# chenghuailin/trajectory_optimization_matrix_lie_groups

Measured on AMD Instinct MI355X. Metric: DDP iterations/sec at batch x horizon = 4096 x 200 (SE3 tracking), higher is better.
Workload: dtype f64

## Files before the change

### trajectory_optimization_matrix_lie_groups_amd/csrc/tolg_backward3.h

```cpp
template <int M>
__host__ __device__ constexpr int urow(int u) { return (u < 3 || M == 6) ? 6 + u : 11; }

#ifndef TOLG_DPP_BUILTIN
#define DF3(acc, p, q, L) "v_fmac_f64_dpp " acc ", " p ", " q " row_newbcast:" L " row_mask:0xf bank_mask:0xf\n\t"
template <int M, int J, int LN>
TOLG_DEV void ldl3_update(double (&a)[M], double w) {
  constexpr int R = M - 1 - J;
  if constexpr (J == 0) {
    if constexpr (M == 6)
      asm volatile("s_nop 1" : "+v"(a[1]), "+v"(a[2]), "+v"(a[3]), "+v"(a[4]), "+v"(a[5]));
    else
      asm volatile("s_nop 1" : "+v"(a[1]), "+v"(a[2]), "+v"(a[3]));
  }
  if constexpr (R == 5)
    asm volatile(DF3("%0", "%0", "%5", "%6") DF3("%1", "%1", "%5", "%6") DF3("%2", "%2", "%5", "%6")
                     DF3("%3", "%3", "%5", "%6") DF3("%4", "%4", "%5", "%6")
                 : "+v"(a[J + 1]), "+v"(a[J + 2]), "+v"(a[J + 3]), "+v"(a[J + 4]), "+v"(a[J + 5]) : "v"(w), "n"(LN));
  if constexpr (R == 4)
    asm volatile(DF3("%0", "%0", "%4", "%5") DF3("%1", "%1", "%4", "%5") DF3("%2", "%2", "%4", "%5")
                     DF3("%3", "%3", "%4", "%5")
                 : "+v"(a[J + 1]), "+v"(a[J + 2]), "+v"(a[J + 3]), "+v"(a[J + 4]) : "v"(w), "n"(LN));
  if constexpr (R == 3)
    asm volatile(DF3("%0", "%0", "%3", "%4") DF3("%1", "%1", "%3", "%4") DF3("%2", "%2", "%3", "%4")
                 : "+v"(a[J + 1]), "+v"(a[J + 2]), "+v"(a[J + 3]) : "v"(w), "n"(LN));
// ... 120 lines not shown
  ldl3_tie_columns<M>(a);
  zn[0] = y[0] * nri[0];
  if constexpr (M > 1) { ldl3_fwd_row<M, 1, LO>(y[1], a[1], zn); zn[1] = y[1] * nri[1]; }
  if constexpr (M > 2) { ldl3_fwd_row<M, 2, LO>(y[2], a[2], zn); zn[2] = y[2] * nri[2]; }
  if constexpr (M > 3) { ldl3_fwd_row<M, 3, LO>(y[3], a[3], zn); zn[3] = y[3] * nri[3]; }
  if constexpr (M > 4) { ldl3_fwd_row<M, 4, LO>(y[4], a[4], zn); zn[4] = y[4] * nri[4]; }
  if constexpr (M > 5) { ldl3_fwd_row<M, 5, LO>(y[5], a[5], zn); zn[5] = y[5] * nri[5]; }
}
template <int M, int LO = 0>
TOLG_DEV void ldl3_backward_nx(const double (&a)[M], const double (&nri)[M], double (&y)[M], const double (&zn)[M], double (&nx)[M]) {
  nx[M - 1] = zn[M - 1];
  if constexpr (M > 1) { ldl3_bwd_row<M, M - 2, urow<M>(M - 2) + LO>(y[M - 2], a, nx); nx[M - 2] = y[M - 2] * nri[M - 2]; }
  if constexpr (M > 2) { ldl3_bwd_row<M, M - 3, urow<M>(M - 3) + LO>(y[M - 3], a, nx); nx[M - 3] = y[M - 3] * nri[M - 3]; }
  if constexpr (M > 3) { ldl3_bwd_row<M, M - 4, urow<M>(M - 4) + LO>(y[M - 4], a, nx); nx[M - 4] = y[M - 4] * nri[M - 4]; }
  if constexpr (M > 4) { ldl3_bwd_row<M, M - 5, urow<M>(M - 5) + LO>(y[M - 5], a, nx); nx[M - 5] = y[M - 5] * nri[M - 5]; }
  if constexpr (M > 5) { ldl3_bwd_row<M, M - 6, urow<M>(M - 6) + LO>(y[M - 6], a, nx); nx[M - 6] = y[M - 6] * nri[M - 6]; }
}

enum { B3_DATA = 5120, B3_ZBYTES = 256,
       B3_ID = B3_DATA + B3_ZBYTES, B3_IDBYTES = 6 * 192, B3_SLOT = B3_ID + B3_IDBYTES,
       B3_TRS = 14, B3_TR = 2 * B3_SLOT, B3_TRBYTES = 4 * 12 * B3_TRS * 8, B3_DUMP = B3_TR + B3_TRBYTES,
       B3_KC = B3_DUMP + 12 * B3_TRS * 8, B3_LDS = B3_KC + 16 * 16 * 8 };

template <int M, bool GRAV, bool AL, bool FAST = false, bool PTW = false>
__global__ __launch_bounds__(64) void k_backward3(Params P, int it, int flags) {
  if ((flags & 4) && !P.k2_redo[blockIdx.x]) return;
  const int ms = flags & 1;
  const bool closed = (flags & 2) != 0;
  const DConsts& C = *(const DConsts*)P.c;
  const int lane = threadIdx.x, g = lane >> 4, j = lane & 15;
  const int b = blockIdx.x * 4 + g;
  const bool act = P.active[b] != 0;
  if constexpr (FAST) {
    const bool back = __any(act && P.mu[b] != 0.0) || P.k2_hint[blockIdx.x] != 0;
    if (lane == 0) P.k2_redo[blockIdx.x] = back ? 1 : 0;
    if (back) return;
  }
  if (!__any(act)) return;
  const int N = P.N;
  __shared__ __attribute__((aligned(16))) char lds[FAST ? (B3_LDS > 34 * 1024 ? B3_LDS : 34 * 1024) : B3_LDS];
  if (lane < B3_ZBYTES / 8) {
    reinterpret_cast<double*>(lds + B3_DATA)[lane] = 0.0;
    reinterpret_cast<double*>(lds + B3_SLOT + B3_DATA)[lane] = 0.0;
  }
  for (int k = lane; k < B3_IDBYTES / 8; k += 64) {
    const int c6 = k / 24, w = k % 24, pr = w / 8, hf = w % 8;
    const double v = (hf < 2 && 2 * pr + hf == c6) ? 1.0 : 0.0;
    reinterpret_cast<double*>(lds + B3_ID)[k] = v;
    reinterpret_cast<double*>(lds + B3_SLOT + B3_ID)[k] = v;
  }
  __builtin_amdgcn_wave_barrier();
  const unsigned lds0 = (unsigned)(uintptr_t)(__attribute__((address_space(3))) char*)lds;

  const double m12 = (j < 12) ? 1.0 : 0.0;
  int mycol = -1;
#pragma unroll
  for (int u = 0; u < M; u++) if (j == urow<M>(u)) mycol = u;
  double bu[M], ibu[M];
#pragma unroll
  for (int u = 0; u < M; u++) { bu[u] = fu_entry<M>(*P.c, urow<M>(u) - 6, u); ibu[u] = 1.0 / bu[u]; }
  double kBW[6], Rt[M], wm[M];
  if constexpr (PTW) {
    const double wd = (j >= 6 && j < 12) ? C.wts[(size_t)(WT_W2 + (j >= 6 && j < 12 ? j - 6 : 0)) * P.Bp + b] : 0.0;
#pragma unroll
    for (int r = 0; r < 6; r++) kBW[r] = (j >= 6 && j < 12) ? 2.0 * (r == j - 6 ? wd : 0.0) : 0.0;
  } else {
#pragma unroll
    for (int r = 0; r < 6; r++) kBW[r] = (j >= 6 && j < 12) ? 2.0 * C.W2[6 * r + (j - 6)] : 0.0;
  }
  {
    double ibc = 0.0;
#pragma unroll
    for (int u = 0; u < M; u++) if (mycol == u) ibc = ibu[u];
    const double rd = (PTW && mycol >= 0) ? C.wts[(size_t)(WT_R + (mycol >= 0 ? mycol : 0)) * P.Bp + b] : 0.0;
#pragma unroll
    for (int u = 0; u < M; u++) {
      Rt[u] = (mycol >= 0) ? 2.0 * (PTW ? (u == mycol ? rd : 0.0) : C.R[u * M + (mycol >= 0 ? mycol : 0)]) * ibu[u] * ibc : 0.0;
      wm[u] = (mycol > u) ? 1.0 : 0.0;
    }
  }
  int fT = REC_D, fM = REC_D + 3;
  bool hT = false, hM = false;
  if (j < 3) { fT = REC_RI + 3 * j; fM = REC_TRI + 3 * j; hT = true; hM = true; }
  else if (j < 6) { fM = REC_RI + 3 * (j - 3); hM = true; }
  else if (j < 9) { fT = REC_JR + 3 * (j - 6); fM = REC_QR + 3 * (j - 6); hT = true; hM = true; }
  else if (j < 12) { fM = REC_JR + 3 * (j - 9); hM = true; }
  else if (j == 12 && !closed) { hT = true; hM = true; }
  const bool vcol = j >= 6 && j < 12;
  const bool hasB = (j == 12 && !closed), isVec = (j == 12 || j == 13);
  const int fB = REC_D + 6;
  const bool hL = (j < 6 || isVec);
  const unsigned lg = (unsigned)g * 16u;
  const unsigned ZP = (unsigned)B3_DATA;
  unsigned oT[3], oM[3], oL[6];
#pragma unroll
  for (int r = 0; r < 3; r++) { oT[r] = hT ? lg + FOFF(fT + r) : ZP; oM[r] = hM ? lg + FOFF(fM + r) : ZP; }
#pragma unroll
  for (int r = 0; r < 6; r++) oL[r] = hL ? lg + FOFF((j < 6) ? REC_LXX + sym6(r, j) : REC_LX + r) : ZP;
  const unsigned oB = hasB ? lg + FOFF(fB) : vcol ? (unsigned)B3_ID + (unsigned)(j - 6) * 192u : ZP;
  unsigned oXA = lg + FOFF(REC_XI), oXB = oXA;
  {
    double aA[2] = {0, 0}, bA[2] = {0, 0}, aB[2] = {0, 0}, bB[2] = {0, 0}, mA[3] = {0, 0, 0}, mB[3] = {0, 0, 0};
    if (vcol) {
      const Consts& G = *P.c;
      const int Cb = (j - 6) / 3, cc = (j - 6) % 3, kA = (cc + 1) % 3, kB = (cc + 2) % 3;
      auto sg = [](int r, int c) { return ((c - r + 3) % 3 == 1) ? -1.0 : 1.0; };
      const double dt = G.dt, ms = G.mass;
      const double iaA = G.Ibinv[4 * kA], iaB = G.Ibinv[4 * kB], icA = G.Jvinv[4 * kA], icB = G.Jvinv[4 * kB];
      const double a_kA = G.Ib[4 * kA], a_kB = G.Ib[4 * kB], a_cc = G.Ib[4 * cc], c_cc = G.Jv[4 * cc];
      const double sA = sg(kA, cc), sB_ = sg(kB, cc);
      if (so3_family(G.kind)) {
        if (Cb == 0) { aA[0] = dt * iaA * sA * (a_kB - a_cc); aB[0] = dt * iaB * sB_ * (a_kA - a_cc); }
      } else if (Cb == 0) {
        aA[0] = dt * iaA * sA * a_kB; bA[0] = -dt * iaA * sA * a_cc;
        aB[0] = dt * iaB * sB_ * a_kA; bB[0] = -dt * iaB * sB_ * a_cc;
        bA[1] = dt * icA * sA * ms; bB[1] = dt * icB * sB_ * ms;
      } else {
        aA[0] = -dt * iaA * sA * c_cc; bA[0] = dt * iaA * sA * ms;
        aB[0] = -dt * iaB * sB_ * c_cc; bB[0] = dt * iaB * sB_ * ms;
        bA[1] = -dt * icA * sA * c_cc; bB[1] = -dt * icB * sB_ * c_cc;
      }
      mA[kA] = 1.0; mB[kB] = 1.0;
      oXA = lg + FOFF(REC_XI + 2 * kA); oXB = lg + FOFF(REC_XI + 2 * kB);
    }
    if (g == 0) {
      double* kc = reinterpret_cast<double*>(lds + B3_KC) + 16 * j;
      kc[0] = aA[0]; kc[1] = bA[0]; kc[2] = aB[0]; kc[3] = bB[0]; kc[4] = bA[1]; kc[5] = bB[1];
#pragma unroll
      for (int r = 0; r < 3; r++) { kc[6 + 2 * r] = mA[r]; kc[7 + 2 * r] = mB[r]; }
    }
  }
  const unsigned oKC = (unsigned)B3_KC + 128u * (unsigned)j;
  const unsigned oV = isVec ? lg + FOFF(REC_LX + 6) : ZP;
  const unsigned oU = isVec ? lg + FOFF(REC_LU) : ZP;
  const unsigned oG = lg + FOFF(REC_LU + M);
  constexpr bool al = AL;
  constexpr unsigned blockBytes = (unsigned)rec_fields(M, GRAV, AL, false) * 32u;
  constexpr int NKB = (int)((blockBytes + 1023u) / 1024u);
  static_assert(NKB == 3 || NKB == 4, "record block of four trajectories: 3 or 4 KB");
  const unsigned oUU = (al && mycol >= 0) ? lg + FOFF(P.fLUU + (mycol >= 0 ? mycol : 0)) : ZP;
  const unsigned wTR = (j < 12) ? (unsigned)B3_TR + ((unsigned)g * 12u * B3_TRS + (unsigned)j) * 8u : (unsigned)B3_DUMP;
  const unsigned rTR = (j < 12) ? (unsigned)B3_TR + ((unsigned)g * 12u * B3_TRS + (unsigned)j * B3_TRS) * 8u : ZP;
  const double hsym = (j < 12) ? 0.5 : 1.0;
  const unsigned sB = (unsigned)P.Bp * 8u;
  const unsigned vr = REC_VR(b);
  const unsigned vG = GK_VG(b, M) + GOFF(0, (j < 13 ? j : 12), M);
  const size_t recStride = (size_t)P.recF * P.Bp, gStride = (size_t)13 * M * P.Bp;
  double Cg[GRAV ? 3 : 1][6];
  if constexpr (GRAV) {
#pragma unroll
    for (int a = 0; a < 3; a++)
#pragma unroll
      for (int r = 0; r < 6; r++) Cg[a][r] = (j < 3) ? C.Llin[a][6 * r + (j < 3 ? j : 0)] : 0.0;
  }
  double mu = P.mu[b], delta = P.delta[b];
  int warned = 0;

  auto dma_from = [&](const char* src, int s) {
    const unsigned dst = (unsigned)__builtin_amdgcn_readfirstlane((int)(lds0 + (unsigned)s * B3_SLOT));
    if constexpr (NKB == 3) rl_dma16x3_rec(uniform_ptr(src), (unsigned)lane * 16u, dst);
    else rl_dma16x4_rec(uniform_ptr(src), (unsigned)lane * 16u, dst);
  };
  auto dma_knot = [&](int i, int s) {
    dma_from(reinterpret_cast<const char*>(P.REC + recStride * i) + (size_t)blockIdx.x * blockBytes, s);
  };
  const char* rec_run = reinterpret_cast<const char*>(P.REC + recStride * (size_t)(N > 2 ? N - 2 : 0)) + (size_t)blockIdx.x * blockBytes;
  const double* gk_run = P.GK + gStride * (size_t)(N + 1);
  const size_t recStrideB = recStride * 8;

  double V[12];
  {
    __amdgpu_buffer_rsrc_t rR = mkbuf(P.REC + recStride * N, (unsigned)P.recF * sB);
    const unsigned OOB = 0x40000000u;
    const double pd = (PTW && j >= 6 && j < 12) ? C.wts[(size_t)(WT_P2 + (j >= 6 && j < 12 ? j - 6 : 0)) * P.Bp + b] : 0.0;
#pragma unroll
    for (int r = 0; r < 6; r++) {
      const int fl = (j < 6) ? REC_LXX + sym6(r, j) : REC_LX + r;
      double t1 = bld(rR, hL ? vr + FOFF(fl) : OOB, 0), t2 = bld(rR, isVec ? vr + FOFF(REC_LX + 6 + r) : OOB, 0);
      V[r] = t1;
      double p2 = (j >= 6 && j < 12) ? 2.0 * (PTW ? (r == j - 6 ? pd : 0.0) : C.P2[6 * r + (j - 6)]) : 0.0;
      V[6 + r] = t2 + p2;
    }
  }
  double gsum = 0;
  double Kst[M];
#pragma unroll
  for (int u = 0; u < M; u++) Kst[u] = 0;
  auto store_gains = [&](const double* gk) {
    if (act && j < 13) {
      __amdgpu_buffer_rsrc_t rGs = mkbuf(gk, 13 * M * sB);
#pragma unroll
      for (int u = 0; u < M; u += 2) bst2_gk(rGs, vG, GOFF(u, 0, M), Kst[u], Kst[u + 1]);
    }
  };
#ifdef TOLG_STAMPS
  unsigned long long st_acc[8] = {0, 0, 0, 0, 0, 0, 0, 0}, st_t = __builtin_amdgcn_s_memtime();
  const unsigned long long st_rt0 = __builtin_amdgcn_s_memrealtime(), st_ct0 = st_t;
#endif

  bool failed = false;
  auto step = [&](int i, auto slot_tag) {
    constexpr int SLOT = decltype(slot_tag)::value;
    const char* sl = lds + SLOT * B3_SLOT;
    auto ld = [&](unsigned off) -> double { return *reinterpret_cast<const double*>(sl + off); };
    auto ld2 = [&](unsigned off, int k, double& x0, double& x1) {
      const f64x2 w = *reinterpret_cast<const f64x2*>(sl + off + k * 64);
      x0 = w.x; x1 = w.y;
    };
    if (i == 0) asm volatile("s_waitcnt vmcnt(0)" ::: "memory");
    else asm volatile("s_waitcnt vmcnt(%0)" :: "n"(M / 2 + NKB) : "memory");
    double A[12], Qh[12], lu[M], luu_i = 0.0;
#pragma unroll
    for (int r = 0; r < 3; r++) { A[r] = ld(oT[r]); A[3 + r] = ld(oM[r]); }
#pragma unroll
    for (int r = 0; r < 6; r += 2) ld2(oB, r / 2, A[6 + r], A[7 + r]);
#pragma unroll
    for (int r = 0; r < 6; r++) Qh[r] = ld(oL[r]);
#pragma unroll
    for (int r = 0; r < 6; r += 2) ld2(oV, r / 2, Qh[6 + r], Qh[7 + r]);
#pragma unroll
    for (int a = 0; a < M; a += 2) ld2(oU, a / 2, lu[a], lu[a + 1]);
    if constexpr (al) luu_i = ld(oUU);
    if constexpr (GRAV) {
      double gv[3];
#pragma unroll
      for (int a = 0; a < 3; a++) gv[a] = *reinterpret_cast<const double*>(sl + oG + (FOFF(REC_LU + M + a) - FOFF(REC_LU + M)));
#pragma unroll
      for (int r = 0; r < 6; r++) A[6 + r] += gv[0] * Cg[0][r] + gv[1] * Cg[1][r] + gv[2] * Cg[2][r];
    }
    const f64x2 xA = *reinterpret_cast<const f64x2*>(sl + oXA), xB = *reinterpret_cast<const f64x2*>(sl + oXB);
    const f64x2* kc = reinterpret_cast<const f64x2*>(lds + oKC);
    const f64x2 c0 = kc[0], c1 = kc[1], c2 = kc[2];
    const f64x2 mk0 = kc[3], mk1 = kc[4], mk2 = kc[5];
    STAMP(0)
    double Z[12];
#pragma unroll
    for (int r = 0; r < 12; r++) Z[r] = (1.0 - m12) * V[r];
    rank1_bk3_0(Z, V, A[0], A[1], A[2]); rank1_bk3_3_nn(Z, V, A[3], A[4], A[5]);
    {
      const double eA0 = fma(c0.x, xB.x, c0.y * xB.y), eB0 = fma(c1.x, xA.x, c1.y * xA.y), eA1 = c2.x * xB.y, eB1 = c2.y * xA.y;
      A[6] = fma(mk0.y, eB0, fma(mk0.x, eA0, A[6])); A[9] = fma(mk0.y, eB1, fma(mk0.x, eA1, A[9]));
      A[7] = fma(mk1.y, eB0, fma(mk1.x, eA0, A[7])); A[10] = fma(mk1.y, eB1, fma(mk1.x, eA1, A[10]));
      A[8] = fma(mk2.y, eB0, fma(mk2.x, eA0, A[8])); A[11] = fma(mk2.y, eB1, fma(mk2.x, eA1, A[11]));
    }
    rank1_bk3_6_nn(Z, V, A[6], A[7], A[8]); rank1_bk3_9_nn(Z, V, A[9], A[10], A[11]);
    STAMP(1)
    __builtin_amdgcn_sched_barrier(0);
    asm volatile("s_waitcnt lgkmcnt(0)" ::: "memory");
#ifdef TOLG_STAMPS2
    STAMP(1)
#endif
    gk_run -= gStride;
    if (i < N - 1) store_gains(gk_run);
#ifdef TOLG_STAMPS2
    STAMP(2)
#endif
    rec_run -= recStrideB;
    if (i >= 2) dma_from(rec_run, SLOT);
    __builtin_amdgcn_sched_barrier(0);
#ifndef TOLG_STAMPS2
    STAMP(2)
#endif
    bool use_lu = false;
    double mu_used = 0.0;
    auto build = [&](double mu_, double (&Gm)[M], double (&Mt)[M]) {
      const double muA = m12 * mu_;
#pragma unroll
      for (int u = 0; u < M; u++) {
        Gm[u] = fma(lu[u], ibu[u], Z[urow<M>(u)]);
        Mt[u] = V[urow<M>(u)] + Rt[u];
      }
      if (__any(mu_ != 0.0)) {
#pragma unroll
        for (int u = 0; u < M; u++) {
          Gm[u] = fma(muA, A[urow<M>(u)], Gm[u]);
          Mt[u] += (mycol == u) ? mu_ : 0.0;
// ... 32 lines not shown
#define TOLG_K3_SYMP 4
#endif
    static_assert(TOLG_K3_SYMP >= 1 && (TOLG_K3_SYMP & (TOLG_K3_SYMP - 1)) == 0, "symmetrisation period: a power of two");
    constexpr int SYMP = FAST ? TOLG_K3_SYMP : 1;
    const bool sym_now = SYMP == 1 || (SLOT == 0 && (SYMP == 2 || (i & (SYMP - 1)) == 0));
    if (sym_now) {
#pragma unroll
      for (int r = 0; r < 12; r++) *reinterpret_cast<double*>(lds + wTR + r * (B3_TRS * 8)) = Qh[r];
    }
    double T[12];
    auto read_T = [&]() {
#pragma unroll
      for (int k = 0; k < 6; k++) {
        const f64x2 t = *reinterpret_cast<const f64x2*>(lds + rTR + 16 * k);
        T[2 * k] = t.x; T[2 * k + 1] = t.y;
      }
    };
    auto symmetrise = [&]() {
      if (!sym_now) return;
      read_T();
#pragma unroll
      for (int r = 0; r < 12; r++) Qh[r] = hsym * (Qh[r] + T[r]);
    };
    auto grad_term = [&](const double (&G)[M]) {
      double s0 = 0, s1 = 0;
#pragma unroll
      for (int u = 0; u < M; u += 2) {
        const double q0 = bu[u] * G[u], q1 = bu[u + 1] * G[u + 1];
        s0 = fma(q0, q0, s0); s1 = fma(q1, q1, s1);
      }
      const double s_ = s0 + s1;
      const double y = __builtin_amdgcn_rsq(s_);
      const double r_ = s_ * y, h_ = 0.5 * y;
      const double rt = fma(h_, fma(-r_, r_, s_), r_);
      gsum += (s_ > 0.0) ? rt : 0.0;
    };
    auto finish = [&](double (&Y)[M], const double (&Uf)[M], double (&nri)[M]) {
      grad_term(Y);
      STAMP(4)
      if (!ms) {
#pragma unroll
        for (int u = 0; u < M; u++) nri[u] = (j == 13) ? 0.0 : nri[u];
      }
      double zn[M], nx[M];
      ldl3_forward<M>(Uf, nri, Y, zn);
      symmetrise();
      STAMP(5)
      if constexpr (M == 6) rank1_bi_x6_nn(Qh, Y, zn);
      else rank1_bi_x4_nn(Qh, Y, zn);
      ldl3_backward_nx<M>(Uf, nri, Y, zn, nx);
#pragma unroll
      for (int u = 0; u < M; u++) Kst[u] = ibu[u] * nx[u];
    };
    bool settled = false;
#ifdef TOLG_K3_NOFAST
    if (false) {
#else
    if (FAST || !__any(act && mu != 0.0)) {
#endif
      double Y[M], Uf[M], nri[M], dv[M];
#pragma unroll
      for (int u = 0; u < M; u++) {
        Y[u] = fma(lu[u], ibu[u], Z[urow<M>(u)]);
        Uf[u] = V[urow<M>(u)] + Rt[u];
        if constexpr (al) Uf[u] += (mycol == u) ? luu_i * ibu[u] * ibu[u] : 0.0;
      }
      ldl3_factor<M>(Uf, nri, dv, wm);
      const bool pd = ldl3_all_positive<M>(dv);
      STAMP(3)
      if (!__any(act && !pd)) {
        if (act) { delta = fmin(1.0, delta) * 0.5; mu = 0.0; }
        finish(Y, Uf, nri);
        settled = true;
      }
    }
    if constexpr (FAST) {
      if (!settled) { failed = true; return; }
    } else if (!settled) {
      double Y2[M], U2[M], nr2[M], d2[M];
      for (;;) {
        if (!done) {
          mu_used = mu;
          build(mu, Y2, U2);
          ldl3_factor<M>(U2, nr2, d2, wm);
          done = schedule(ldl3_all_positive<M>(d2));
        }
        if (__all(done)) break;
      }
      build(mu_used, Y2, U2);
      ldl3_factor<M>(U2, nr2, d2, wm);
      if (!__any(use_lu)) {
        finish(Y2, U2, nr2);
      } else {
        double Gk[M], Mc[M], Ac[M][M], Xl[M], zn[M], nx[M];
        build(mu_used, Gk, Mc);
        grad_term(Gk);
// ... 32 lines not shown
#pragma unroll
        for (int u = 0; u < M; u++) Kst[u] = ibu[u] * (use_lu ? -((j == 13) ? 0.0 : Xl[u]) : nx[u]);
      }
    }
#pragma unroll
    for (int r = 0; r < 12; r++) V[r] = Qh[r];
    STAMP(6)
  };

  dma_knot(N - 1, (N - 1) & 1);
  if (N >= 2) dma_knot(N - 2, (N - 2) & 1);
  asm volatile("s_waitcnt vmcnt(0)" ::: "memory");
  int i = N - 1;
  if (i & 1) { step(i, std::integral_constant<int, 1>()); i--; }
  for (; i >= 1 && !(FAST && failed); i -= 2) {
    step(i, std::integral_constant<int, 0>());
    if (FAST && failed) break;
    step(i - 1, std::integral_constant<int, 1>());
  }
  if (i == 0 && !(FAST && failed)) step(0, std::integral_constant<int, 0>());
  if constexpr (FAST) {
    if (failed) {
      asm volatile("s_waitcnt vmcnt(0)" ::: "memory");
      if (lane == 0) { P.k2_redo[blockIdx.x] = 1; P.k2_hint[blockIdx.x] = 8; }
      return;
    }
  } else {
    const bool anyf = __any(failed);
    if (lane == 0) { const int hn = (it == 0) ? 0 : P.k2_hint[blockIdx.x]; P.k2_hint[blockIdx.x] = anyf ? 8 : (hn > 0 ? hn - 1 : 0); }
  }
  store_gains(P.GK);
#ifdef TOLG_STAMPS
  STAMP(7)
  if (blockIdx.x == 7 && lane == 0 && P.mu_hist) {
    for (int k = 0; k < 8; k++) P.mu_hist[(size_t)28 * P.max_iter + k] = (double)st_acc[k];
    P.mu_hist[(size_t)29 * P.max_iter + 0] = (double)(__builtin_amdgcn_s_memrealtime() - st_rt0);
    P.mu_hist[(size_t)29 * P.max_iter + 1] = (double)(__builtin_amdgcn_s_memtime() - st_ct0);
  }
#endif
  double grad = (ms ? bcast<12>(gsum) : bcast<13>(gsum)) / (double)N;
  if (act && j == 0) {
    P.mu[b] = mu;
    P.delta[b] = delta;
    P.grad[b] = grad;
    if (warned) P.status[b] = TOLG_ST_MAXREG;
    if (it >= 0 && b < P.B) {
      if (P.grad_hist) P.grad_hist[(size_t)b * (P.max_iter + 1) + it] = grad;
      if (P.mu_hist && it < P.max_iter) P.mu_hist[(size_t)b * P.max_iter + it] = mu;
    }
    if (it >= 0) {
      bool conv = ms ? (grad < P.tol_grad && P.dn[b] < P.tol_defect) : (grad < P.tol_grad);
      if (conv) { P.conv[b] = 1; P.active[b] = 0; }
    }
  }
}
```

### trajectory_optimization_matrix_lie_groups_amd/csrc/tolg_kernels.hip

```cpp
#include <hip/hip_runtime.h>
#include <hip/hip_ext.h>
#include <type_traits>
#include <math.h>
#include <stdint.h>
#include <stdio.h>
#include <stdlib.h>
#include <string.h>
#include <new>
#include <vector>

#include "../../include/tolg.h"
#include "tolg_lie.h"

namespace tolg {

struct Consts {
  int kind, m, N, diagJ;
  double dt, mass, grav, pend_k;
  double J[36], Jinv[36], Ib[9];
  double Jv[9], Ibinv[9], Jvinv[9];
  double W1[36], W2[36], P1[36], P2[36];
  double R[36];
  double Bt[9], Bb[9];
  double Llin[3][36];
// ... 3405 lines not shown
  int b = blockIdx.x * blockDim.x + threadIdx.x;
  if (b >= P.B) return;
  if (J) J[b] = P.Jc[b];
  if (dn) dn[b] = P.dn[b];
  if (grad) grad[b] = P.grad[b];
  if (mu_delta) { mu_delta[2 * b] = P.mu[b]; mu_delta[2 * b + 1] = P.delta[b]; }
  if (iters) iters[b] = P.iters[b];
  if (status) status[b] = P.status[b];
  if (conv) conv[b] = P.conv[b];
}

}

using namespace tolg;

typedef void (*SearchKernel)(Params, int, int, int);
typedef void (*SearchRollout)(Params, int, int, int, int);
struct KernelTable {
  void (*init)(Params, const double*, const double*, const double*, int);
  void (*init_warm)(Params, const double*, const double*, const double*, const double*, const double*);
  void (*linearize)(Params, const double*, const double*, double*, double*, int, int, int, int, int);
  void (*init_rollout)(Params);
  void (*sweep[2][2])(Params, int, int);
  void (*rollout_linear)(Params, double, int, int);
  void (*rollout_alpha1)(Params, double, int, int);
  void (*rollout_factor)(Params, double, int, int);
  void (*rollout_lin)(Params, int);
  void (*ec_ring[2])(Params);
  void (*ec_stmt[2])(Params);
  void (*affine_commit)(Params, int, int);
  void (*policy_rollout)(Params, int, int, const double*, const double*, double*, int*, double*, double*, double*);
  void (*mpc_advance)(Params, const double*, double*, double*, double*, double*, double*, double*);
  void (*policy_rollout_plant[2])(Params, int, int, const double*, const double*, double*, int*, double*, double*, double*, PlantArg);
  void (*mpc_advance_plant[2])(Params, const double*, double*, double*, double*, double*, double*, double*, PlantArg);
  struct Search {
    struct { SearchRollout k; int nt; } wave2[2];
    SearchRollout wave1[2];
    SearchKernel eval_t[2];
    SearchKernel eval, eval_affine;
  } ls[2];
};

template <int M, bool MS, int PK, int PT>
static KernelTable::Search search_kernels() {
  KernelTable::Search s;
  s.wave2[1] = {k_rollout_ls2<M, false, 1, PK>, 1};
  if constexpr (MS || PK == 1) s.wave2[0] = {k_rollout_ls2<M, MS, 1, PK>, 1};
  else s.wave2[0] = {k_rollout_ls2<M, false, 3>, 3};
  s.wave1[0] = k_rollout_ls<M, MS, false, PK>;
  s.wave1[1] = k_rollout_ls<M, MS, true, PK>;
  s.eval_t[0] = k_rollout_eval_t<M, MS, false, PT>;
  s.eval_t[1] = k_rollout_eval_t<M, MS, true, PT>;
  s.eval = k_ls_eval<M, MS, PT>;
  s.eval_affine = k_ls_eval_affine<M, MS, PT>;
  return s;
}
template <int M, bool GRAV, bool DENSE, bool PEND, int PT>
static KernelTable kernel_table(int lds_per_block) {
  constexpr int PK = PEND ? 1 : 0;
  constexpr bool PTREF = (PT & PT_REF) != 0, PTW = (PT & PT_W) != 0;
  KernelTable t;
  t.init = k_init<PTREF>;
  t.init_warm = k_init_warm;
  t.linearize = k_linearize<M, PT>;
  t.init_rollout = k_init_rollout<M>;
  if constexpr (!DENSE && !PEND) {
    t.sweep[0][0] = k_backward3<M, GRAV, false, false, PTW>; t.sweep[0][1] = k_backward3<M, GRAV, true, false, PTW>;
    t.sweep[1][0] = k_backward3<M, GRAV, false, true, PTW>;  t.sweep[1][1] = k_backward3<M, GRAV, true, true, PTW>;
  } else {
    t.sweep[0][0] = t.sweep[0][1] = k_backward<M, PEND, GRAV, PEND && !DENSE, false, PTW>;
    t.sweep[1][0] = t.sweep[1][1] = k_backward<M, PEND, GRAV, PEND && !DENSE, true, PTW>;
  }
  t.rollout_linear = k_rollout<M, true, false>;
  t.rollout_alpha1 = k_rollout<M, false, true, PK>;
  t.rollout_factor = k_rollout<M, false, false, PK>;
  t.rollout_lin = nullptr;
  if constexpr (!PEND)
    if (rl_static_lds<M>() + sizeof(double) * RL_NH * 4 * 16 <= (size_t)lds_per_block) t.rollout_lin = k_rollout_lin<M, PT>;
  t.ec_ring[0] = k_expected_change_ring<M, GRAV, false, DENSE || PEND, PEND, PTW>;
  t.ec_ring[1] = k_expected_change_ring<M, GRAV, true, DENSE || PEND, PEND, PTW>;
  t.ec_stmt[0] = k_expected_change<M, PK, false, PTW>;
  t.ec_stmt[1] = k_expected_change<M, PK, true, PTW>;
  t.affine_commit = k_affine_commit<M>;
  t.policy_rollout = k_policy_rollout<M, PK, PT & ~PT_OBS>;
  t.mpc_advance = k_mpc_advance<M, PK, PT & ~PT_OBS>;
  t.policy_rollout_plant[TOLG_PLANT_DIAG] = k_policy_rollout<M, PK, PT & ~PT_OBS, PL_DIAG, PlantArg>;
  t.policy_rollout_plant[TOLG_PLANT_DENSE] = k_policy_rollout<M, PK, PT & ~PT_OBS, PL_DENSE, PlantArg>;
  t.mpc_advance_plant[TOLG_PLANT_DIAG] = k_mpc_advance<M, PK, PT & ~PT_OBS, PL_DIAG, PlantArg>;
  t.mpc_advance_plant[TOLG_PLANT_DENSE] = k_mpc_advance<M, PK, PT & ~PT_OBS, PL_DENSE, PlantArg>;
  t.ls[0] = search_kernels<M, false, PK, PT>();
  t.ls[1] = search_kernels<M, true, PK, PT>();
// ... 60 lines not shown
  Params P;
  Params run;
  tolg_options run_opt;
  LsPlan run_ls;
  int run_it;
  bool running;
  int lds_per_block;
  int rec_closed = 0;
  KernelTable kt;
  KernelTable kt_pt[8];
  const double* ref_shared;
  const double* refs = nullptr;
  int refs_B = 0;
  const double* wts = nullptr;
  int wts_B = 0;
  const double* obs = nullptr;
  int obs_B = 0, obs_K = 0;
  double *obs_lam = nullptr, *obs_imu = nullptr;
  const double* plant = nullptr;
  int plant_B = 0, plant_S = 0, plant_form = 0;
  int pol_B = 0;
  bool pol_traj_fast = false;
  bool k2_full_only, ls_one_wave;
  const double *al_lb, *al_ub, *al_lambda, *al_imu;
  LazyRes cnt;
  LazyRes side;
  bool timing;
  std::vector<hipEvent_t> ev;
  std::vector<int> ev_kind;
  size_t ev_used;
};

static size_t align_up(size_t x, size_t a) { return (x + a - 1) / a * a; }
static int padded_batch(int B) { return (B + 3) / 4 * 4; }
static dim3 traj_grid(const Params& P) { return dim3((P.Bp + 63) / 64); }
static dim3 knot_grid(int knots, int Bp) { return dim3((unsigned)(((size_t)knots * Bp + 255) / 256)); }

static bool batch_fits(const tolg_handle_s* h, int B) {
  return B >= 1 && B <= h->max_batch && !(h->refs && B != h->refs_B) && !(h->wts && B != h->wts_B) && !(h->obs && B != h->obs_B);
}
static void select_kernels(tolg_handle_s* h) {
  h->kt = h->kt_pt[(h->refs ? PT_REF : 0) | (h->wts ? PT_W : 0) | (h->obs ? PT_OBS : 0)];
}

static int host_inv6(const double A[36], double Ai[36]) {
  double Mx[6][12];
// ... 173 lines not shown
        double sacc = 0;
        if (j < 3 && c.grav != 0.0 && prob->kind != TOLG_DYN_PENDULUM3D)
          for (int k = 0; k < 3; k++) sacc += c.Jinv[6 * i + 3 + k] * S[3 * k + j];
        if (j < 3 && i < 3 && prob->kind == TOLG_DYN_PENDULUM3D) {
          const double SS[9] = {c.pend_k * S[3 + 0], c.pend_k * S[3 + 1], c.pend_k * S[3 + 2],
                                -c.pend_k * S[0], -c.pend_k * S[1], -c.pend_k * S[2], 0, 0, 0};
          for (int k = 0; k < 3; k++) sacc += c.Ibinv[3 * i + k] * SS[3 * k + j];
        }
        c.Llin[a][6 * i + j] = sacc * prob->dt;
      }
  }
  h->kt_pt[0] = kernel_table_for<0>(*prob, c, h->lds_per_block);
  h->kt_pt[PT_REF] = kernel_table_for<PT_REF>(*prob, c, h->lds_per_block);
  h->kt_pt[PT_W] = kernel_table_for<PT_W>(*prob, c, h->lds_per_block);
  h->kt_pt[PT_REF | PT_W] = kernel_table_for<PT_REF | PT_W>(*prob, c, h->lds_per_block);
  h->kt_pt[PT_OBS] = kernel_table_for<PT_OBS>(*prob, c, h->lds_per_block);
  h->kt_pt[PT_REF | PT_OBS] = kernel_table_for<PT_REF | PT_OBS>(*prob, c, h->lds_per_block);
  h->kt_pt[PT_W | PT_OBS] = kernel_table_for<PT_W | PT_OBS>(*prob, c, h->lds_per_block);
  h->kt_pt[PT_REF | PT_W | PT_OBS] = kernel_table_for<PT_REF | PT_W | PT_OBS>(*prob, c, h->lds_per_block);
  select_kernels(h);
  {
    const char* e = getenv("TOLG_K2_FULL_ONLY");
    h->k2_full_only = e && e[0] == '1';
    e = getenv("TOLG_LS_ONEWAVE");
    h->ls_one_wave = e && e[0] == '1';
    e = getenv("TOLG_POLICY_TRAJ_FAST");
    h->pol_traj_fast = e && e[0] == '1';
  }
  hipStream_t st = static_cast<hipStream_t>(stream);
  memset(&h->P, 0, sizeof h->P);
  carve_all(prob, h->Bp_max, h->ws, h->P);
  h->P.N = prob->N; h->P.m = prob->m;
  h->ref_shared = h->P.ref;
  Consts* dc = const_cast<Consts*>(h->P.c);
  if (hipMemcpyAsync(dc, &h->hc, sizeof(Consts), hipMemcpyHostToDevice, st) != hipSuccess) { tolg_destroy(h); return TOLG_E_LAUNCH; }
  int N = prob->N;
  hipLaunchKernelGGL(k_pack_ref, dim3((N + 1 + 63) / 64), dim3(64), 0, st, N, d_q_ref, d_xi_ref,
                     const_cast<double*>(h->P.ref));
  LAUNCH_CHECK();
  *out = h;
  return 0;
}

extern "C" void tolg_destroy(tolg_handle_t h) {
  if (!h) return;
  h->cnt.release();
  h->side.release();
  for (auto e : h->ev) (void)hipEventDestroy(e);
  delete h;
}

extern "C" void tolg_enable_timing(tolg_handle_t h, int32_t on) {
  if (!h) return;
  h->timing = on != 0;
  if (h->timing && h->ev.empty()) {
    h->ev.resize(2 * 1024);
    for (auto& e : h->ev) (void)hipEventCreate(&e);
    h->ev_kind.resize(1024);
  }
  h->ev_used = 0;
}

namespace {
struct Timed {
  tolg_handle_s* h; hipStream_t st; int kind; bool on, ext;
  bool count = true;
  Timed(tolg_handle_s* h_, hipStream_t s, int k, bool ext_ = false) : h(h_), st(s), kind(k), ext(ext_) {
    on = h->timing;
// ... 57 lines not shown
  return P;
}

static int run_linearize(tolg_handle_s* h, const Params& P, hipStream_t st, const double* src, const double* src_u,
                         double* dst, double* dst_u, int ms, int i0 = 0, int ni = -1, int ls_list = -1, int ls_nslots = 0,
                         decltype(KernelTable::linearize) kernel = nullptr) {
  if (ni < 0) ni = P.N + 1;
  h->rec_closed = 0;
  Timed t(h, st, 2);
  hipLaunchKernelGGL(kernel ? kernel : h->kt.linearize, knot_grid(ni, P.Bp), dim3(256), 0, st, P, src, src_u, dst, dst_u, ms, i0,
                     ni, ls_list, ls_nslots);
  LAUNCH_CHECK();
  return 0;
}
static int run_backward(tolg_handle_s* h, const Params& P, hipStream_t st, int it, int ms) {
  ms = (ms ? 1 : 0) | (h->rec_closed ? 2 : 0);
  const dim3 grid(P.Bp / 4), blk(64);
  const bool al = P.al_lb != nullptr;
  const bool fast = it > 0 && !h->k2_full_only;
  for (int pass = fast ? 0 : 1; pass < 2; pass++) {
    Timed t(h, st, 0, true);
    t.count = (pass == 0) || !fast;
    const int fl = ms | ((pass == 1 && fast) ? 4 : 0);
    t.launch(h->kt.sweep[pass == 0][al], grid, blk, P, it, fl);
    LAUNCH_CHECK();
  }
  return 0;
}
static int run_rollout_ms(tolg_handle_s* h, const Params& P, hipStream_t st, double alpha, int linear, int ms = 1,
                          int i0 = 0, int i1 = -1) {
  if (i1 < 0) i1 = P.N;
  Timed t(h, st, 1);
  dim3 grid((P.Bp * 4 + 63) / 64), blk(64);
  const KernelTable& T = h->kt;
  hipLaunchKernelGGL(linear ? T.rollout_linear : (alpha == 1.0 || !ms) ? T.rollout_alpha1 : T.rollout_factor, grid, blk, 0,
                     st, P, alpha, i0, i1);
  LAUNCH_CHECK();
  return 0;
}
static void launch_ec_ring(const tolg_handle_s* h, const Params& P, hipStream_t st, bool store) {
  hipLaunchKernelGGL(h->kt.ec_ring[store], dim3(P.Bp / 4), dim3(64), 0, st, P);
}
static void launch_ec_stmt(const tolg_handle_s* h, const Params& P, hipStream_t st, bool redo) {
  hipLaunchKernelGGL(h->kt.ec_stmt[redo], dim3((P.Bp * 4 + 63) / 64), dim3(64), 0, st, P);
}
static int run_affine_dev(tolg_handle_s* h, const Params& P, hipStream_t st, bool merit) {
  Timed t(h, st, 1);
// ... 673 lines not shown
```

Before: 1823.

## Pair fast backward sweep waves with helper waves computing gains via LDS ring

```diff
diff --git a/trajectory_optimization_matrix_lie_groups_amd/csrc/tolg_backward3.h b/trajectory_optimization_matrix_lie_groups_amd/csrc/tolg_backward3.h
--- a/trajectory_optimization_matrix_lie_groups_amd/csrc/tolg_backward3.h
+++ b/trajectory_optimization_matrix_lie_groups_amd/csrc/tolg_backward3.h
@@ -166,35 +166,84 @@
        B3_TRS = 14, B3_TR = 2 * B3_SLOT, B3_TRBYTES = 4 * 12 * B3_TRS * 8, B3_DUMP = B3_TR + B3_TRBYTES,
        B3_KC = B3_DUMP + 12 * B3_TRS * 8, B3_LDS = B3_KC + 16 * 16 * 8 };
 
-template <int M, bool GRAV, bool AL, bool FAST = false, bool PTW = false>
-__global__ __launch_bounds__(64) void k_backward3(Params P, int it, int flags) {
-  if ((flags & 4) && !P.k2_redo[blockIdx.x]) return;
+typedef rl_sync_t b3_sync_t;
+enum { B3_STOP = -1 };
+TOLG_DEV int b3_wait(b3_sync_t p, int v) {
+  int x = *p;
+  for (int n = 0; n < RL_POLLS && x >= 0 && x < v; n++) {
+    __builtin_amdgcn_s_sleep(2);
+    x = *p;
+  }
+  return x;
+}
+template <int M>
+struct B3Ring { enum { ROWS = 3 * M / 2, SLOT = ROWS * 1024, BYTES = 2 * SLOT }; };
+template <int M>
+TOLG_DEV void b3_ring_put_factor(char* rs, const double (&a)[M], const double (&nri)[M], double s_) {
+  f64x2* q = reinterpret_cast<f64x2*>(rs);
+#pragma unroll
+  for (int u = 0; u < M; u += 2) q[(u / 2) * 64] = f64x2{nri[u], nri[u + 1]};
+#pragma unroll
+  for (int u = 1; u < M; u += 2) q[(M / 2 + u / 2) * 64] = f64x2{a[u], u + 1 < M ? a[u + 1 < M ? u + 1 : u] : s_};
+}
+template <int M>
+TOLG_DEV void b3_ring_put_y(char* rs, const double (&Y)[M]) {
+  f64x2* q = reinterpret_cast<f64x2*>(rs);
+#pragma unroll
+  for (int u = 0; u < M; u += 2) q[(M + u / 2) * 64] = f64x2{Y[u], Y[u + 1]};
+}
+TOLG_DEV double b3_grad_root(double s_) {
+  const double y = __builtin_amdgcn_rsq(s_);
+  const double r_ = s_ * y, h_ = 0.5 * y;
+  const double rt = fma(h_, fma(-r_, r_, s_), r_);
+  return (s_ > 0.0) ? rt : 0.0;
+}
+TOLG_DEV void b3_epilogue_grad(const Params& P, int it, int ms, int b, bool act, int j, double gsum) {
+  double grad = (ms ? bcast<12>(gsum) : bcast<13>(gsum)) / (double)P.N;
+  if (act && j == 0) {
+    P.grad[b] = grad;
+    if (it >= 0 && b < P.B && P.grad_hist) P.grad_hist[(size_t)b * (P.max_iter + 1) + it] = grad;
+    if (it >= 0) {
+      bool conv = ms ? (grad < P.tol_grad && P.dn[b] < P.tol_defect) : (grad < P.tol_grad);
+      if (conv) { P.conv[b] = 1; P.active[b] = 0; }
+    }
+  }
+}
+
+struct B3Pair {
+  unsigned ring;
+  b3_sync_t prod, cons;
+};
+template <int M, bool GRAV, bool AL, bool FAST, bool PTW, int ROLE>
+TOLG_DEV void b3_sweep(const Params& P, const int it, const int flags, const int grp, char* const lds, const unsigned wb, const B3Pair pr) {
+  static_assert(ROLE == 0 || FAST, "only the fast sweep has a helper");
+  auto leave = [&]() { if constexpr (ROLE == 1) *pr.prod = B3_STOP; };
+  if ((flags & 4) && !P.k2_redo[grp]) { leave(); return; }
   const int ms = flags & 1;
   const bool closed = (flags & 2) != 0;
   const DConsts& C = *(const DConsts*)P.c;
-  const int lane = threadIdx.x, g = lane >> 4, j = lane & 15;
-  const int b = blockIdx.x * 4 + g;
+  const int lane = threadIdx.x & 63, g = lane >> 4, j = lane & 15;
+  const int b = grp * 4 + g;
   const bool act = P.active[b] != 0;
   if constexpr (FAST) {
-    const bool back = __any(act && P.mu[b] != 0.0) || P.k2_hint[blockIdx.x] != 0;
-    if (lane == 0) P.k2_redo[blockIdx.x] = back ? 1 : 0;
-    if (back) return;
-  }
-  if (!__any(act)) return;
+    const bool back = __any(act && P.mu[b] != 0.0) || P.k2_hint[grp] != 0;
+    if (lane == 0) P.k2_redo[grp] = back ? 1 : 0;
+    if (back) { leave(); return; }
+  }
+  if (!__any(act)) { leave(); return; }
   const int N = P.N;
-  __shared__ __attribute__((aligned(16))) char lds[FAST ? (B3_LDS > 34 * 1024 ? B3_LDS : 34 * 1024) : B3_LDS];
   if (lane < B3_ZBYTES / 8) {
-    reinterpret_cast<double*>(lds + B3_DATA)[lane] = 0.0;
-    reinterpret_cast<double*>(lds + B3_SLOT + B3_DATA)[lane] = 0.0;
+    reinterpret_cast<double*>(lds + wb + B3_DATA)[lane] = 0.0;
+    reinterpret_cast<double*>(lds + wb + B3_SLOT + B3_DATA)[lane] = 0.0;
   }
   for (int k = lane; k < B3_IDBYTES / 8; k += 64) {
     const int c6 = k / 24, w = k % 24, pr = w / 8, hf = w % 8;
     const double v = (hf < 2 && 2 * pr + hf == c6) ? 1.0 : 0.0;
-    reinterpret_cast<double*>(lds + B3_ID)[k] = v;
-    reinterpret_cast<double*>(lds + B3_SLOT + B3_ID)[k] = v;
+    reinterpret_cast<double*>(lds + wb + B3_ID)[k] = v;
+    reinterpret_cast<double*>(lds + wb + B3_SLOT + B3_ID)[k] = v;
   }
   __builtin_amdgcn_wave_barrier();
-  const unsigned lds0 = (unsigned)(uintptr_t)(__attribute__((address_space(3))) char*)lds;
+  const unsigned lds0 = (unsigned)(uintptr_t)(__attribute__((address_space(3))) char*)lds + wb;
 
   const double m12 = (j < 12) ? 1.0 : 0.0;
   int mycol = -1;
@@ -234,14 +283,14 @@
   const bool hasB = (j == 12 && !closed), isVec = (j == 12 || j == 13);
   const int fB = REC_D + 6;
   const bool hL = (j < 6 || isVec);
-  const unsigned lg = (unsigned)g * 16u;
-  const unsigned ZP = (unsigned)B3_DATA;
+  const unsigned lg = wb + (unsigned)g * 16u;
+  const unsigned ZP = wb + (unsigned)B3_DATA;
   unsigned oT[3], oM[3], oL[6];
 #pragma unroll
   for (int r = 0; r < 3; r++) { oT[r] = hT ? lg + FOFF(fT + r) : ZP; oM[r] = hM ? lg + FOFF(fM + r) : ZP; }
 #pragma unroll
   for (int r = 0; r < 6; r++) oL[r] = hL ? lg + FOFF((j < 6) ? REC_LXX + sym6(r, j) : REC_LX + r) : ZP;
-  const unsigned oB = hasB ? lg + FOFF(fB) : vcol ? (unsigned)B3_ID + (unsigned)(j - 6) * 192u : ZP;
+  const unsigned oB = hasB ? lg + FOFF(fB) : vcol ? wb + (unsigned)B3_ID + (unsigned)(j - 6) * 192u : ZP;
   unsigned oXA = lg + FOFF(REC_XI), oXB = oXA;
   {
     double aA[2] = {0, 0}, bA[2] = {0, 0}, aB[2] = {0, 0}, bB[2] = {0, 0}, mA[3] = {0, 0, 0}, mB[3] = {0, 0, 0};
@@ -268,13 +317,13 @@
       oXA = lg + FOFF(REC_XI + 2 * kA); oXB = lg + FOFF(REC_XI + 2 * kB);
     }
     if (g == 0) {
-      double* kc = reinterpret_cast<double*>(lds + B3_KC) + 16 * j;
+      double* kc = reinterpret_cast<double*>(lds + wb + B3_KC) + 16 * j;
       kc[0] = aA[0]; kc[1] = bA[0]; kc[2] = aB[0]; kc[3] = bB[0]; kc[4] = bA[1]; kc[5] = bB[1];
 #pragma unroll
       for (int r = 0; r < 3; r++) { kc[6 + 2 * r] = mA[r]; kc[7 + 2 * r] = mB[r]; }
     }
   }
-  const unsigned oKC = (unsigned)B3_KC + 128u * (unsigned)j;
+  const unsigned oKC = wb + (unsigned)B3_KC + 128u * (unsigned)j;
   const unsigned oV = isVec ? lg + FOFF(REC_LX + 6) : ZP;
   const unsigned oU = isVec ? lg + FOFF(REC_LU) : ZP;
   const unsigned oG = lg + FOFF(REC_LU + M);
@@ -283,8 +332,8 @@
   constexpr int NKB = (int)((blockBytes + 1023u) / 1024u);
   static_assert(NKB == 3 || NKB == 4, "record block of four trajectories: 3 or 4 KB");
   const unsigned oUU = (al && mycol >= 0) ? lg + FOFF(P.fLUU + (mycol >= 0 ? mycol : 0)) : ZP;
-  const unsigned wTR = (j < 12) ? (unsigned)B3_TR + ((unsigned)g * 12u * B3_TRS + (unsigned)j) * 8u : (unsigned)B3_DUMP;
-  const unsigned rTR = (j < 12) ? (unsigned)B3_TR + ((unsigned)g * 12u * B3_TRS + (unsigned)j * B3_TRS) * 8u : ZP;
+  const unsigned wTR = wb + ((j < 12) ? (unsigned)B3_TR + ((unsigned)g * 12u * B3_TRS + (unsigned)j) * 8u : (unsigned)B3_DUMP);
+  const unsigned rTR = (j < 12) ? wb + (unsigned)B3_TR + ((unsigned)g * 12u * B3_TRS + (unsigned)j * B3_TRS) * 8u : ZP;
   const double hsym = (j < 12) ? 0.5 : 1.0;
   const unsigned sB = (unsigned)P.Bp * 8u;
   const unsigned vr = REC_VR(b);
@@ -306,9 +355,9 @@
     else rl_dma16x4_rec(uniform_ptr(src), (unsigned)lane * 16u, dst);
   };
   auto dma_knot = [&](int i, int s) {
-    dma_from(reinterpret_cast<const char*>(P.REC + recStride * i) + (size_t)blockIdx.x * blockBytes, s);
+    dma_from(reinterpret_cast<const char*>(P.REC + recStride * i) + (size_t)grp * blockBytes, s);
   };
-  const char* rec_run = reinterpret_cast<const char*>(P.REC + recStride * (size_t)(N > 2 ? N - 2 : 0)) + (size_t)blockIdx.x * blockBytes;
+  const char* rec_run = reinterpret_cast<const char*>(P.REC + recStride * (size_t)(N > 2 ? N - 2 : 0)) + (size_t)grp * blockBytes;
   const double* gk_run = P.GK + gStride * (size_t)(N + 1);
   const size_t recStrideB = recStride * 8;
 
@@ -343,6 +392,8 @@
 #endif
 
   bool failed = false;
+  bool stuck = false;
+  const unsigned oR = pr.ring + (unsigned)lane * 16u;
   auto step = [&](int i, auto slot_tag) {
     constexpr int SLOT = decltype(slot_tag)::value;
     const char* sl = lds + SLOT * B3_SLOT;
@@ -352,7 +403,7 @@
       x0 = w.x; x1 = w.y;
     };
     if (i == 0) asm volatile("s_waitcnt vmcnt(0)" ::: "memory");
-    else asm volatile("s_waitcnt vmcnt(%0)" :: "n"(M / 2 + NKB) : "memory");
+    else asm volatile("s_waitcnt vmcnt(%0)" :: "n"((ROLE == 1 ? 0 : M / 2) + NKB) : "memory");
     double A[12], Qh[12], lu[M], luu_i = 0.0;
 #pragma unroll
     for (int r = 0; r < 3; r++) { A[r] = ld(oT[r]); A[3 + r] = ld(oM[r]); }
@@ -390,12 +441,14 @@
     rank1_bk3_6_nn(Z, V, A[6], A[7], A[8]); rank1_bk3_9_nn(Z, V, A[9], A[10], A[11]);
     STAMP(1)
     __builtin_amdgcn_sched_barrier(0);
+    int cons_seen = 0;
+    if constexpr (ROLE == 1) cons_seen = *pr.cons;
     asm volatile("s_waitcnt lgkmcnt(0)" ::: "memory");
 #ifdef TOLG_STAMPS2
     STAMP(1)
 #endif
     gk_run -= gStride;
-    if (i < N - 1) store_gains(gk_run);
+    if constexpr (ROLE == 0) { if (i < N - 1) store_gains(gk_run); }
 #ifdef TOLG_STAMPS2
     STAMP(2)
 #endif
@@ -474,6 +527,7 @@
 #pragma unroll
       for (int r = 0; r < 12; r++) Qh[r] = hsym * (Qh[r] + T[r]);
     };
+    double ring_s = 0.0;
     auto grad_term = [&](const double (&G)[M]) {
       double s0 = 0, s1 = 0;
 #pragma unroll
@@ -482,10 +536,8 @@
         s0 = fma(q0, q0, s0); s1 = fma(q1, q1, s1);
       }
       const double s_ = s0 + s1;
-      const double y = __builtin_amdgcn_rsq(s_);
-      const double r_ = s_ * y, h_ = 0.5 * y;
-      const double rt = fma(h_, fma(-r_, r_, s_), r_);
-      gsum += (s_ > 0.0) ? rt : 0.0;
+      if constexpr (ROLE == 1) { ring_s = s_; return; }
+      gsum += b3_grad_root(s_);
     };
     auto finish = [&](double (&Y)[M], const double (&Uf)[M], double (&nri)[M]) {
       grad_term(Y);
@@ -495,14 +547,27 @@
         for (int u = 0; u < M; u++) nri[u] = (j == 13) ? 0.0 : nri[u];
       }
       double zn[M], nx[M];
+      char* const rs = lds + oR + SLOT * B3Ring<M>::SLOT;
+      if constexpr (ROLE == 1) {
+        const int need = N - 2 - i;
+        if (__builtin_amdgcn_readfirstlane(cons_seen) < need && b3_wait(pr.cons, need) < need) { stuck = true; return; }
+        b3_ring_put_factor<M>(rs, Uf, nri, ring_s);
+      }
       ldl3_forward<M>(Uf, nri, Y, zn);
+      if constexpr (ROLE == 1) {
+        b3_ring_put_y<M>(rs, Y);
+        asm volatile("" ::: "memory");
+        *pr.prod = N - i;
+      }
       symmetrise();
       STAMP(5)
       if constexpr (M == 6) rank1_bi_x6_nn(Qh, Y, zn);
       else rank1_bi_x4_nn(Qh, Y, zn);
-      ldl3_backward_nx<M>(Uf, nri, Y, zn, nx);
-#pragma unroll
-      for (int u = 0; u < M; u++) Kst[u] = ibu[u] * nx[u];
+      if constexpr (ROLE == 0) {
+        ldl3_backward_nx<M>(Uf, nri, Y, zn, nx);
+#pragma unroll
+        for (int u = 0; u < M; u++) Kst[u] = ibu[u] * nx[u];
+      }
     };
     bool settled = false;
 #ifdef TOLG_K3_NOFAST
@@ -523,7 +588,7 @@
       if (!__any(act && !pd)) {
         if (act) { delta = fmin(1.0, delta) * 0.5; mu = 0.0; }
         finish(Y, Uf, nri);
-        settled = true;
+        settled = !stuck;
       }
     }
     if constexpr (FAST) {
@@ -602,35 +667,131 @@
   if constexpr (FAST) {
     if (failed) {
       asm volatile("s_waitcnt vmcnt(0)" ::: "memory");
-      if (lane == 0) { P.k2_redo[blockIdx.x] = 1; P.k2_hint[blockIdx.x] = 8; }
+      leave();
+      if (stuck) { if (act && j == 0) P.status[b] = TOLG_ST_INTERNAL; return; }
+      if (lane == 0) { P.k2_redo[grp] = 1; P.k2_hint[grp] = 8; }
       return;
     }
   } else {
     const bool anyf = __any(failed);
-    if (lane == 0) { const int hn = (it == 0) ? 0 : P.k2_hint[blockIdx.x]; P.k2_hint[blockIdx.x] = anyf ? 8 : (hn > 0 ? hn - 1 : 0); }
-  }
-  store_gains(P.GK);
+    if (lane == 0) { const int hn = (it == 0) ? 0 : P.k2_hint[grp]; P.k2_hint[grp] = anyf ? 8 : (hn > 0 ? hn - 1 : 0); }
+  }
+  if constexpr (ROLE == 0) store_gains(P.GK);
 #ifdef TOLG_STAMPS
   STAMP(7)
-  if (blockIdx.x == 7 && lane == 0 && P.mu_hist) {
+  if (grp == 7 && lane == 0 && P.mu_hist) {
     for (int k = 0; k < 8; k++) P.mu_hist[(size_t)28 * P.max_iter + k] = (double)st_acc[k];
     P.mu_hist[(size_t)29 * P.max_iter + 0] = (double)(__builtin_amdgcn_s_memrealtime() - st_rt0);
     P.mu_hist[(size_t)29 * P.max_iter + 1] = (double)(__builtin_amdgcn_s_memtime() - st_ct0);
   }
 #endif
-  double grad = (ms ? bcast<12>(gsum) : bcast<13>(gsum)) / (double)N;
   if (act && j == 0) {
     P.mu[b] = mu;
     P.delta[b] = delta;
-    P.grad[b] = grad;
     if (warned) P.status[b] = TOLG_ST_MAXREG;
-    if (it >= 0 && b < P.B) {
-      if (P.grad_hist) P.grad_hist[(size_t)b * (P.max_iter + 1) + it] = grad;
-      if (P.mu_hist && it < P.max_iter) P.mu_hist[(size_t)b * P.max_iter + it] = mu;
-    }
-    if (it >= 0) {
-      bool conv = ms ? (grad < P.tol_grad && P.dn[b] < P.tol_defect) : (grad < P.tol_grad);
-      if (conv) { P.conv[b] = 1; P.active[b] = 0; }
-    }
-  }
-}
+    if (it >= 0 && b < P.B && P.mu_hist && it < P.max_iter) P.mu_hist[(size_t)b * P.max_iter + it] = mu;
+  }
+  if constexpr (ROLE == 0) b3_epilogue_grad(P, it, ms, b, act, j, gsum);
+}
+
+template <int M>
+TOLG_DEV void b3_helper(const Params& P, const int it, const int flags, const int grp, char* const lds, const B3Pair pr) {
+  const int ms = flags & 1;
+  const int lane = threadIdx.x & 63, g = lane >> 4, j = lane & 15;
+  const int b = grp * 4 + g;
+  const bool act = P.active[b] != 0;
+  const int N = P.N;
+  double ibu[M];
+#pragma unroll
+  for (int u = 0; u < M; u++) ibu[u] = 1.0 / fu_entry<M>(*P.c, urow<M>(u) - 6, u);
+  const unsigned sB = (unsigned)P.Bp * 8u;
+  const unsigned vG = GK_VG(b, M) + GOFF(0, (j < 13 ? j : 12), M);
+  const size_t gStride = (size_t)13 * M * P.Bp;
+  const double* gk = P.GK + gStride * (size_t)N;
+  const char* const ring = lds + pr.ring + (unsigned)lane * 16u;
+  double gsum = 0;
+  for (int i = N - 1; i >= 0; i--) {
+    const int k = N - i;
+    const int seen = b3_wait(pr.prod, k);
+    if (seen < k) {
+      if (seen >= 0 && act && j == 0) P.status[b] = TOLG_ST_INTERNAL;
+      return;
+    }
+    asm volatile("" ::: "memory");
+    const f64x2* q = reinterpret_cast<const f64x2*>(ring + (i & 1) * B3Ring<M>::SLOT);
+    double a[M], nri[M], Y[M], zn[M], nx[M], s_ = 0.0;
+    a[0] = 0.0;
+#pragma unroll
+    for (int u = 0; u < M; u += 2) { const f64x2 w = q[(u / 2) * 64]; nri[u] = w.x; nri[u + 1] = w.y; }
+#pragma unroll
+    for (int u = 1; u < M; u += 2) {
+      const f64x2 w = q[(M / 2 + u / 2) * 64];
+      a[u] = w.x;
+      if (u + 1 < M) a[u + 1 < M ? u + 1 : u] = w.y; else s_ = w.y;
+    }
+#pragma unroll
+    for (int u = 0; u < M; u += 2) { const f64x2 w = q[(M + u / 2) * 64]; Y[u] = w.x; Y[u + 1] = w.y; }
+    asm volatile("s_waitcnt lgkmcnt(0)" ::: "memory");
+    *pr.cons = k;
+#pragma unroll
+    for (int u = 0; u < M; u++) zn[u] = 0.0;
+    zn[M - 1] = Y[M - 1] * nri[M - 1];
+    ldl3_tie_columns<M>(a);
+    ldl3_backward_nx<M>(a, nri, Y, zn, nx);
+    gk -= gStride;
+    if (act && j < 13) {
+      __amdgpu_buffer_rsrc_t rGs = mkbuf(gk, 13 * M * sB);
+#pragma unroll
+      for (int u = 0; u < M; u += 2) bst2_gk(rGs, vG, GOFF(u, 0, M), ibu[u] * nx[u], ibu[u + 1] * nx[u + 1]);
+    }
+    gsum += b3_grad_root(s_);
+  }
+  b3_epilogue_grad(P, it, ms, b, act, j, gsum);
+}
+
+template <int M, bool GRAV, bool AL, bool FAST = false, bool PTW = false>
+__global__ __launch_bounds__(64) void k_backward3(Params P, int it, int flags) {
+  __shared__ __attribute__((aligned(16))) char lds[FAST ? (B3_LDS > 34 * 1024 ? B3_LDS : 34 * 1024) : B3_LDS];
+  b3_sweep<M, GRAV, AL, FAST, PTW, 0>(P, it, flags, (int)blockIdx.x, lds, 0u, B3Pair{0u, nullptr, nullptr});
+}
+
+#ifndef TOLG_K2_NOHELPER
+template <int M, bool GRAV, bool AL, bool PTW>
+__global__ __launch_bounds__(512) void k_backward3h(Params P, int it, int flags, unsigned* stats) {
+  enum { RING0 = 4 * B3_LDS, SYNC = RING0 + 4 * B3Ring<M>::BYTES };
+  __shared__ __attribute__((aligned(16))) char lds[SYNC + 64];
+  static_assert(SYNC + 64 <= 160 * 1024, "four sweep waves and their rings: one CU's LDS");
+  const b3_sync_t sync = (b3_sync_t)(__attribute__((address_space(3))) char*)(lds + SYNC);
+  const int w = __builtin_amdgcn_readfirstlane((int)(threadIdx.x >> 6));
+  const int simd = (int)__builtin_amdgcn_s_getreg(4 | (4 << 6) | (1 << 11));
+  if (threadIdx.x >= 8 && threadIdx.x < 16) sync[threadIdx.x] = 0;
+  if ((threadIdx.x & 63) == 0) sync[w] = simd;
+  __syncthreads();
+  int sid[8];
+#pragma unroll
+  for (int v = 0; v < 8; v++) sid[v] = __builtin_amdgcn_readfirstlane(sync[v]);
+  bool paired = (flags & 8) == 0;
+  int rank = 0;
+#pragma unroll
+  for (int v = 0; v < 8; v++) {
+    int c = 0;
+#pragma unroll
+    for (int u = 0; u < 8; u++) c += (sid[u] == sid[v]) ? 1 : 0;
+    paired = paired && c == 2;
+    rank += (sid[v] == simd && v < w) ? 1 : 0;
+  }
+  if (stats && threadIdx.x == 0) atomicAdd(&stats[paired ? 0 : 1], 1u);
+  const int groups = P.Bp / 4;
+  if (paired) {
+    const int grp = (int)blockIdx.x * 4 + simd;
+    if (grp >= groups) return;
+    const B3Pair pr{(unsigned)RING0 + (unsigned)simd * (unsigned)B3Ring<M>::BYTES, sync + 8 + 2 * simd, sync + 9 + 2 * simd};
+    if (rank == 0) b3_sweep<M, GRAV, AL, true, PTW, 1>(P, it, flags, grp, lds, (unsigned)simd * (unsigned)B3_LDS, pr);
+    else b3_helper<M>(P, it, flags, grp, lds, pr);
+  } else {
+    const int grp = (int)blockIdx.x * 4 + w;
+    if (w >= 4 || grp >= groups) return;
+    b3_sweep<M, GRAV, AL, true, PTW, 0>(P, it, flags, grp, lds, (unsigned)w * (unsigned)B3_LDS, B3Pair{0u, nullptr, nullptr});
+  }
+}
+#endif
diff --git a/trajectory_optimization_matrix_lie_groups_amd/csrc/tolg_kernels.hip b/trajectory_optimization_matrix_lie_groups_amd/csrc/tolg_kernels.hip
--- a/trajectory_optimization_matrix_lie_groups_amd/csrc/tolg_kernels.hip
+++ b/trajectory_optimization_matrix_lie_groups_amd/csrc/tolg_kernels.hip
@@ -3451,6 +3451,7 @@
   void (*linearize)(Params, const double*, const double*, double*, double*, int, int, int, int, int);
   void (*init_rollout)(Params);
   void (*sweep[2][2])(Params, int, int);
+  void (*sweep_pair[2])(Params, int, int, unsigned*);
   void (*rollout_linear)(Params, double, int, int);
   void (*rollout_alpha1)(Params, double, int, int);
   void (*rollout_factor)(Params, double, int, int);
@@ -3489,6 +3490,7 @@
   constexpr int PK = PEND ? 1 : 0;
   constexpr bool PTREF = (PT & PT_REF) != 0, PTW = (PT & PT_W) != 0;
   KernelTable t;
+  t.sweep_pair[0] = t.sweep_pair[1] = nullptr;
   t.init = k_init<PTREF>;
   t.init_warm = k_init_warm;
   t.linearize = k_linearize<M, PT>;
@@ -3496,6 +3498,9 @@
   if constexpr (!DENSE && !PEND) {
     t.sweep[0][0] = k_backward3<M, GRAV, false, false, PTW>; t.sweep[0][1] = k_backward3<M, GRAV, true, false, PTW>;
     t.sweep[1][0] = k_backward3<M, GRAV, false, true, PTW>;  t.sweep[1][1] = k_backward3<M, GRAV, true, true, PTW>;
+#ifndef TOLG_K2_NOHELPER
+    if (lds_per_block >= 160 * 1024) { t.sweep_pair[0] = k_backward3h<M, GRAV, false, PTW>; t.sweep_pair[1] = k_backward3h<M, GRAV, true, PTW>; }
+#endif
   } else {
     t.sweep[0][0] = t.sweep[0][1] = k_backward<M, PEND, GRAV, PEND && !DENSE, false, PTW>;
     t.sweep[1][0] = t.sweep[1][1] = k_backward<M, PEND, GRAV, PEND && !DENSE, true, PTW>;
@@ -3602,6 +3607,8 @@
   int pol_B = 0;
   bool pol_traj_fast = false;
   bool k2_full_only, ls_one_wave;
+  int k2_pair_mode = 0;
+  unsigned* k2_stats = nullptr;
   const double *al_lb, *al_ub, *al_lambda, *al_imu;
   LazyRes cnt;
   LazyRes side;
@@ -3821,6 +3828,10 @@
   {
     const char* e = getenv("TOLG_K2_FULL_ONLY");
     h->k2_full_only = e && e[0] == '1';
+    e = getenv("TOLG_K2_NOHELPER");
+    h->k2_pair_mode = (e && e[0] == '1') ? 1 : (e && e[0] == '2') ? 2 : 0;
+    e = getenv("TOLG_K2_STATS");
+    if (e && e[0] == '1' && hipMalloc(&h->k2_stats, 2 * sizeof(unsigned)) == hipSuccess) (void)hipMemset(h->k2_stats, 0, 2 * sizeof(unsigned));
     e = getenv("TOLG_LS_ONEWAVE");
     h->ls_one_wave = e && e[0] == '1';
     e = getenv("TOLG_POLICY_TRAJ_FAST");
@@ -3843,6 +3854,12 @@
 
 extern "C" void tolg_destroy(tolg_handle_t h) {
   if (!h) return;
+  if (h->k2_stats) {
+    unsigned n[2] = {0, 0};
+    if (hipMemcpy(n, h->k2_stats, sizeof n, hipMemcpyDeviceToHost) == hipSuccess)
+      fprintf(stderr, "tolg: paired fast sweep: %u workgroups in main / helper pairs, %u on the fall-back path\n", n[0], n[1]);
+    (void)hipFree(h->k2_stats);
+  }
   h->cnt.release();
   h->side.release();
   for (auto e : h->ev) (void)hipEventDestroy(e);
@@ -3946,7 +3963,10 @@
     Timed t(h, st, 0, true);
     t.count = (pass == 0) || !fast;
     const int fl = ms | ((pass == 1 && fast) ? 4 : 0);
-    t.launch(h->kt.sweep[pass == 0][al], grid, blk, P, it, fl);
+    if (pass == 0 && h->kt.sweep_pair[al] && h->k2_pair_mode != 1)
+      t.launch(h->kt.sweep_pair[al], dim3((P.Bp / 4 + 3) / 4), dim3(512), P, it, fl | (h->k2_pair_mode == 2 ? 8 : 0), h->k2_stats);
+    else
+      t.launch(h->kt.sweep[pass == 0][al], grid, blk, P, it, fl);
     LAUNCH_CHECK();
   }
   return 0;
```

Result: slower. 1700 (-6.7%).
